# cxm12/TGSR

Measured on AMD Instinct MI355X. Metric: SR images/sec (32->256, batch 16 per GPU, one step in flight), higher is better.
Workload: dtype f32

## Files before the change

include/tgsr_hip.h:

```cpp
#ifndef TGSR_HIP_H
#define TGSR_HIP_H

#include <stdint.h>

#ifdef __cplusplus
extern "C" {
#endif

#define TGSR_OK 0
#define TGSR_EINVAL (-1)
#define TGSR_EUNSUPPORTED (-2)
#define TGSR_ELAUNCH (-3)

#define TGSR_EPI_AFFINE 0
#define TGSR_EPI_AFFINE_GLU 1

#define TGSR_ACT_NONE 0
#define TGSR_ACT_TANH_AXPY 1
#define TGSR_ACT_IDENT_AXPY 2

#define TGSR_ABI_VERSION 2
int tgsr_abi_version(void);
const char* tgsr_last_error(void);

int64_t tgsr_packed_weight_elems(int Cout, int Cin, int K);
int tgsr_pack_conv_weight(const float* w, float* wpack, int Cout, int Cin, int K, void* stream);
int tgsr_pack_conv_weight_dgrad(const float* w, float* wpack, int Cout, int Cin, int K, void* stream);

int tgsr_bn_fold(const float* weight, const float* bias, const float* running_mean, const float* running_var,
                 float eps, float* scale, float* shift, int C, void* stream);

int tgsr_conv3x3_fwd(const float* x, int64_t x_bstride, int B, int Cin, int H, int W, const float* wpack, int Cout,
                     const float* scale, const float* shift, const float* residual, int64_t res_bstride, float* out,
                     int64_t out_bstride, int epilogue, int upsample, void* stream);
int tgsr_conv3x3_fwd_plan(int B, int H, int W, int Cout, int epilogue, int upsample, int* nob, int* rows_per_wave, int* groups);

int64_t tgsr_packed_upconv_weight_elems(int Cout, int Cin);
int tgsr_pack_upconv_weight(const float* w, float* wpack, int Cout, int Cin, void* stream);
int tgsr_upconv3x3_glu_fwd(const float* x, int64_t x_bstride, int B, int Cin, int H, int W, const float* wpack, int Cout,
                           const float* scale, const float* shift, float* out, int64_t out_bstride, void* stream);

int64_t tgsr_packed_upwino_weight_elems(int Cout, int Cin);
int tgsr_pack_upwino_weight(const float* w, float* upack, int Cout, int Cin, int glu, void* stream);
int tgsr_upwino_glu_fwd(const float* x, int64_t x_bstride, int B, int Cin, int H, int W, const float* upack, int Cout,
                        const float* scale, const float* shift, float* out, int64_t out_bstride, void* stream);
int tgsr_upwino_fwd(const float* x, int64_t x_bstride, int B, int Cin, int H, int W, const float* upack, int Cout,
                    const float* scale, const float* shift, float* out, int64_t out_bstride, void* stream);

int64_t tgsr_packed_upwino4_weight_elems(int Cout, int Cin);
int tgsr_pack_upwino4_weight(const float* w, float* upack, int Cout, int Cin, int glu, void* stream);
int tgsr_upwino4_fwd(const float* x, int64_t x_bstride, int B, int Cin, int H, int W, const float* upack, int Cout,
                     const float* scale, const float* shift, float* out, int64_t out_bstride, int glu, void* stream);

int64_t tgsr_packed_wino_weight_elems(int Cout, int Cin);
int tgsr_pack_wino_weight(const float* w, float* upack, int Cout, int Cin, int glu, void* stream);
int tgsr_pack_wino_weight_dgrad(const float* w, float* upack, int Cout, int Cin, void* stream);
int tgsr_wino_conv3x3_fwd(const float* x, int64_t x_bstride, int B, int Cin, int H, int W, const float* upack, int Cout,
                          const float* scale, const float* shift, const float* residual, int64_t res_bstride,
                          float* out, int64_t out_bstride, int epilogue, void* stream);

int64_t tgsr_packed_wino4_weight_elems(int Cout, int Cin);
int tgsr_pack_wino4_weight(const float* w, float* upack, int Cout, int Cin, int glu, void* stream);
int tgsr_pack_wino4_weight_dgrad(const float* w, float* upack, int Cout, int Cin, void* stream);
int tgsr_wino4_conv3x3_fwd(const float* x, int64_t x_bstride, int B, int Cin, int H, int W, const float* upack, int Cout,
                           const float* scale, const float* shift, const float* residual, int64_t res_bstride,
                           float* out, int64_t out_bstride, int epilogue, void* stream);

int tgsr_pack_wino4_wide_weight(const float* w, float* upack, int Cout, int Cin, int glu, void* stream);
int tgsr_pack_wino4_wide_weight_dgrad(const float* w, float* upack, int Cout, int Cin, void* stream);
int tgsr_wino4_wide_stats_nslots(int B, int H, int W, int Cout);
int tgsr_wino4_wide_conv3x3_stats_fwd(const float* x, int64_t x_bstride, int B, int Cin, int H, int W, const float* upack,
                                      int Cout, float* out, int64_t out_bstride, float* stat_partial, void* stream);
int tgsr_wino4_wide_conv3x3_fwd(const float* x, int64_t x_bstride, int B, int Cin, int H, int W, const float* upack, int Cout,
                                const float* scale, const float* shift, const float* residual, int64_t res_bstride,
                                float* out, int64_t out_bstride, int epilogue, void* stream);

int tgsr_conv_to3_set_pipe(int on);

int tgsr_conv_to3_fwd(const float* x, int64_t x_bstride, int B, int Cin, int H, int W, const float* w, int K,
                      int act, const float* addend, float alpha, float* out, void* stream);
#define TGSR_TO3_FORM_MFMA 0
#define TGSR_TO3_FORM_PIPE 1
#define TGSR_TO3_FORM_VEC4 2
#define TGSR_TO3_FORM_SCALAR 3
int tgsr_conv_to3_plan(const float* x, int64_t x_bstride, int B, int Cin, int H, int W, int K, const float* addend,
                       const float* out, int* form, int* tile_rows);

int tgsr_conv_to3_finish_fwd(const float* x, int64_t x_bstride, int B, int Cin, int H, int W, const float* w, int K, float* out,
                             int n, float* const* fine, const float* const* t, const float* const* s, const int64_t* numel,
                             float alpha, void* stream);

int tgsr_word_attention_fwd(const float* h, int64_t h_bstride, const float* words, const float* w_ctx,
                            const uint8_t* mask, int mask_mode, int B, int idf, int cdf, int T, int Q, float* src_ws,
                            float* c_code, int64_t c_bstride, float* attn, void* stream);

int tgsr_word_project_fwd(const float* words, const float* const* w_ctx, int nsets, int B, int idf, int cdf, int T,
                          float* src_out, void* stream);

int tgsr_bilstm_fwd(const int64_t* captions, int width, const int32_t* cap_lens, int B, int Tmax, const float* emb,
                    int ntoken, int ninput, const float* w_ih, const float* w_hh, const float* b_ih,
                    const float* b_hh, int H, float* gates_ws, float* words_emb, float* sent_emb, void* stream);

int tgsr_lstm_gate_table(const float* emb, int ntoken, int ninput, const float* w_ih, const float* b_ih,
                         const float* b_hh, int H, float* table, void* stream);
int tgsr_bilstm_table_fwd(const int64_t* captions, int width, const int32_t* cap_lens, int B, int Tmax,
                          const float* table, int ntoken, const float* w_hh, int H, float* words_emb, float* sent_emb,
                          void* stream);

int tgsr_gru_gate_table(const float* emb, int ntoken, int ninput, const float* w_ih, const float* b_ih, const float* b_hh_rz,
                        int H, float* table, void* stream);
int tgsr_bigru_table_fwd(const int64_t* captions, int width, const int32_t* cap_lens, int B, int Tmax, const float* table,
                         int ntoken, const float* w_hh, const float* b_hn, int H, float* words_emb, float* sent_emb,
                         void* stream);

int tgsr_bigru_train_fwd(const float* x, const int32_t* cap_lens, int B, int Tmax, int ninput, const float* w_ih,
                         const float* w_hh, const float* b_ih, const float* b_hh_rz, const float* b_hn, int H, float* gates_ws,
                         float* acts, float* words_emb, float* sent_emb, void* stream);
int tgsr_bigru_bwd(const int32_t* cap_lens, int B, int Tmax, int H, const float* w_hh, const float* acts, const float* words_emb,
                   const float* d_words, const float* d_sent, float* dgx, float* dgh, float* hprev, float* dbias, void* stream);

int tgsr_bilstm_train_fwd(const float* x, const int32_t* cap_lens, int B, int Tmax, int ninput, const float* w_ih,
                          const float* w_hh, const float* b_ih, const float* b_hh, int H, float* gates_ws, float* acts,
                          float* words_emb, float* sent_emb, void* stream);
int tgsr_bilstm_bwd(const int32_t* cap_lens, int B, int Tmax, int H, const float* w_hh, const float* acts,
                    const float* words_emb, const float* d_words, const float* d_sent, float* dgates, float* hprev,
                    float* dbias, void* stream);

int tgsr_damsm_words_fwd(const float* words, const int32_t* cap_lens, const float* ctx, int B, int ndf, int Tw, int S,
                         float gamma1, float gamma2, float* sim, float* att_diag, void* stream);

int64_t tgsr_damsm_words_bwd_ws_elems(int B, int ndf, int S);
int tgsr_damsm_words_bwd(const float* words, const int32_t* cap_lens, const float* ctx, const float* grad_sim, int B,
                         int ndf, int Tw, int S, float gamma1, float gamma2, float* ws, float* grad_words32,
                         float* grad_ctx, void* stream);

int tgsr_func_attention_fwd(const float* query, const float* context, int B, int ndf, int L, int S, float gamma1,
                            float* weighted_context, float* attn, void* stream);

int tgsr_conv1x1_fwd(const float* x, int B, int Cin, int S, const float* w, const float* bias, int Cout, float* out,
                     void* stream);
int tgsr_linear_fwd(const float* x, int B, int K, const float* w, const float* bias, int Cout, float* out,
                    void* stream);
// ... 253 lines not shown
```

tgsr_amd/_lib.py:

```python
import ctypes
import os
import subprocess

_HERE = os.path.dirname(os.path.abspath(__file__))
LIB_PATH = os.environ.get("TGSR_LIB_PATH") or os.path.join(_HERE, "lib", "libtgsr_hip.so")
ABI_VERSION = 2

OK, EINVAL, EUNSUPPORTED, ELAUNCH = 0, -1, -2, -3
EPI_AFFINE, EPI_AFFINE_GLU = 0, 1
ACT_NONE, ACT_TANH_AXPY, ACT_IDENT_AXPY = 0, 1, 2
TO3_FORM_MFMA, TO3_FORM_PIPE, TO3_FORM_VEC4, TO3_FORM_SCALAR = 0, 1, 2, 3
DT_BF16, DT_F16 = 1, 2
WGRAD_DIRECT, WGRAD_WINO, WGRAD_UPWINO = 0, 1, 2
WGRAD_FAMILIES = ("conv3x3_wgrad_kernel<%d,%d,%s>", "wino_wgrad_kernel<%d,%d>", "wino_wgrad_dma_kernel<%d>", "upwino_wgrad_kernel<%d>")
WGRAD_PLAN_FIELDS, WGRAD_PLAN_WS = 10, 9
TO3_BWD_PLAN_FIELDS, TO3_BWD_PLAN_WS = 4, 3

_vp, _i, _i64, _f, _d = ctypes.c_void_p, ctypes.c_int, ctypes.c_int64, ctypes.c_float, ctypes.c_double

SIGNATURES = {
    "tgsr_abi_version": (_i, []),
    "tgsr_last_error": (ctypes.c_char_p, []),
    "tgsr_packed_weight_elems": (_i64, [_i, _i, _i]),
    "tgsr_pack_conv_weight": (_i, [_vp, _vp, _i, _i, _i, _vp]),
    "tgsr_pack_conv_weight_dgrad": (_i, [_vp, _vp, _i, _i, _i, _vp]),
    "tgsr_bn_fold": (_i, [_vp, _vp, _vp, _vp, _f, _vp, _vp, _i, _vp]),
    "tgsr_conv3x3_fwd": (_i, [_vp, _i64, _i, _i, _i, _i, _vp, _i, _vp, _vp, _vp, _i64, _vp, _i64, _i, _i, _vp]),
    "tgsr_conv3x3_fwd_plan": (_i, [_i, _i, _i, _i, _i, _i, _vp, _vp, _vp]),
    "tgsr_packed_upconv_weight_elems": (_i64, [_i, _i]),
    "tgsr_pack_upconv_weight": (_i, [_vp, _vp, _i, _i, _vp]),
    "tgsr_upconv3x3_glu_fwd": (_i, [_vp, _i64, _i, _i, _i, _i, _vp, _i, _vp, _vp, _vp, _i64, _vp]),
    "tgsr_packed_upwino_weight_elems": (_i64, [_i, _i]),
    "tgsr_pack_upwino_weight": (_i, [_vp, _vp, _i, _i, _i, _vp]),
    "tgsr_upwino_glu_fwd": (_i, [_vp, _i64, _i, _i, _i, _i, _vp, _i, _vp, _vp, _vp, _i64, _vp]),
    "tgsr_upwino_fwd": (_i, [_vp, _i64, _i, _i, _i, _i, _vp, _i, _vp, _vp, _vp, _i64, _vp]),
    "tgsr_packed_upwino4_weight_elems": (_i64, [_i, _i]),
    "tgsr_pack_upwino4_weight": (_i, [_vp, _vp, _i, _i, _i, _vp]),
    "tgsr_upwino4_fwd": (_i, [_vp, _i64, _i, _i, _i, _i, _vp, _i, _vp, _vp, _vp, _i64, _i, _vp]),
    "tgsr_packed_wino_weight_elems": (_i64, [_i, _i]),
    "tgsr_pack_wino_weight": (_i, [_vp, _vp, _i, _i, _i, _vp]),
    "tgsr_pack_wino_weight_dgrad": (_i, [_vp, _vp, _i, _i, _vp]),
    "tgsr_wino_conv3x3_fwd": (_i, [_vp, _i64, _i, _i, _i, _i, _vp, _i, _vp, _vp, _vp, _i64, _vp, _i64, _i, _vp]),
    "tgsr_packed_wino4_weight_elems": (_i64, [_i, _i]),
    "tgsr_pack_wino4_weight": (_i, [_vp, _vp, _i, _i, _i, _vp]),
    "tgsr_pack_wino4_weight_dgrad": (_i, [_vp, _vp, _i, _i, _vp]),
    "tgsr_pack_wino4_wide_weight": (_i, [_vp, _vp, _i, _i, _i, _vp]),
    "tgsr_pack_wino4_wide_weight_dgrad": (_i, [_vp, _vp, _i, _i, _vp]),
    "tgsr_wino4_wide_stats_nslots": (_i, [_i, _i, _i, _i]),
    "tgsr_wino4_wide_conv3x3_stats_fwd": (_i, [_vp, _i64, _i, _i, _i, _i, _vp, _i, _vp, _i64, _vp, _vp]),
    "tgsr_wino4_wide_conv3x3_fwd": (_i, [_vp, _i64, _i, _i, _i, _i, _vp, _i, _vp, _vp, _vp, _i64, _vp, _i64, _i, _vp]),
    "tgsr_wino4_conv3x3_fwd": (_i, [_vp, _i64, _i, _i, _i, _i, _vp, _i, _vp, _vp, _vp, _i64, _vp, _i64, _i, _vp]),
    "tgsr_conv_to3_fwd": (_i, [_vp, _i64, _i, _i, _i, _i, _vp, _i, _i, _vp, _f, _vp, _vp]),
    "tgsr_conv_to3_plan": (_i, [_vp, _i64, _i, _i, _i, _i, _i, _vp, _vp, _vp, _vp]),
    "tgsr_word_attention_fwd": (_i, [_vp, _i64, _vp, _vp, _vp, _i, _i, _i, _i, _i, _i, _vp, _vp, _i64, _vp, _vp]),
    "tgsr_word_project_fwd": (_i, [_vp, _vp, _i, _i, _i, _i, _i, _vp, _vp]),
    "tgsr_bilstm_fwd": (_i, [_vp, _i, _vp, _i, _i, _vp, _i, _i, _vp, _vp, _vp, _vp, _i, _vp, _vp, _vp, _vp]),
    "tgsr_lstm_gate_table": (_i, [_vp, _i, _i, _vp, _vp, _vp, _i, _vp, _vp]),
    "tgsr_bilstm_table_fwd": (_i, [_vp, _i, _vp, _i, _i, _vp, _i, _vp, _i, _vp, _vp, _vp]),
    "tgsr_bilstm_train_fwd": (_i, [_vp, _vp, _i, _i, _i, _vp, _vp, _vp, _vp, _i, _vp, _vp, _vp, _vp, _vp]),
    "tgsr_bilstm_bwd": (_i, [_vp, _i, _i, _i, _vp, _vp, _vp, _vp, _vp, _vp, _vp, _vp, _vp]),
    "tgsr_damsm_words_fwd": (_i, [_vp, _vp, _vp, _i, _i, _i, _i, _f, _f, _vp, _vp, _vp]),
    "tgsr_damsm_words_bwd_ws_elems": (_i64, [_i, _i, _i]),
    "tgsr_damsm_words_bwd": (_i, [_vp, _vp, _vp, _vp, _i, _i, _i, _i, _f, _f, _vp, _vp, _vp, _vp]),
    "tgsr_func_attention_fwd": (_i, [_vp, _vp, _i, _i, _i, _i, _f, _vp, _vp, _vp]),
    "tgsr_conv1x1_fwd": (_i, [_vp, _i, _i, _i, _vp, _vp, _i, _vp, _vp]),
    "tgsr_linear_fwd": (_i, [_vp, _i, _i, _vp, _vp, _i, _vp, _vp]),
    "tgsr_rowdot_fwd": (_i, [_vp, _vp, _vp, _vp, _i, _i, _vp]),
    "tgsr_ca_net_fwd": (_i, [_vp, _vp, _vp, _vp, _i, _i, _i, _vp, _vp, _vp, _vp]),
    "tgsr_rowdot_bwd": (_i, [_vp, _vp, _vp, _vp, _vp, _i, _i, _vp]),
    "tgsr_bn_train_nsplit": (_i, [_i, _i, _i]),
    "tgsr_bn_train_fwd": (_i, [_vp, _i, _i, _i, _vp, _vp, _f, _f, _vp, _vp, _i, _vp, _i64, _vp, _vp, _vp, _vp, _vp, _vp,
                               _i64, _vp, _vp]),
    "tgsr_bn_train_bwd": (_i, [_vp, _vp, _i, _i, _i, _vp, _vp, _vp, _vp, _i, _vp, _vp, _vp, _vp, _vp, _vp]),
    "tgsr_dconv_set_split": (_i, [_i]),
    "tgsr_bn_set_fuse_small": (_i, [_i]),
    "tgsr_conv_to3_set_pipe": (_i, [_i]),
    "tgsr_conv_to3_finish_fwd": (_i, [_vp, _i64, _i, _i, _i, _i, _vp, _i, _vp, _i, _vp, _vp, _vp, _vp, _f, _vp]),
    "tgsr_conv4x4s2_split_form": (_i, [_i, _i, _i, _i, _i, _i]),
    "tgsr_conv3x3_gemm_split_form": (_i, [_i, _i, _i, _i, _i, _i]),
    "tgsr_conv4x4s2_ws_elems": (_i64, [_i, _i, _i, _i, _i, _i]),
    "tgsr_conv4x4s2_fwd": (_i, [_vp, _i, _i, _i, _i, _vp, _i, _i, _vp, _vp, _vp]),
    "tgsr_conv4x4s2_dgrad": (_i, [_vp, _i, _i, _i, _i, _vp, _i, _vp, _vp, _vp]),
    "tgsr_conv4x4s2_wgrad": (_i, [_vp, _vp, _i, _i, _i, _i, _i, _vp, _vp, _vp]),
    "tgsr_conv3x3_gemm_ws_elems": (_i64, [_i, _i, _i, _i, _i, _i]),
    "tgsr_conv3x3_gemm_fwd": (_i, [_vp, _i, _i, _i, _i, _vp, _i, _vp, _vp, _vp]),
    "tgsr_conv3x3_gemm_dgrad": (_i, [_vp, _i, _i, _i, _i, _vp, _i, _vp, _vp, _vp]),
    "tgsr_conv3x3_gemm_wgrad": (_i, [_vp, _vp, _i, _i, _i, _i, _i, _vp, _vp, _vp]),
    "tgsr_leaky_relu": (_i, [_vp, _vp, _vp, _i64, _vp]),
    "tgsr_glu": (_i, [_vp, _vp, _vp, _i64, _i64, _vp]),
    "tgsr_wino_stats_nslots": (_i, [_i, _i, _i, _i]),
    "tgsr_wino_conv3x3_stats_fwd": (_i, [_vp, _i64, _i, _i, _i, _i, _vp, _i, _vp, _i64, _vp, _vp]),
    "tgsr_wino4_stats_nslots": (_i, [_i, _i, _i, _i]),
    "tgsr_wino4_conv3x3_stats_fwd": (_i, [_vp, _i64, _i, _i, _i, _i, _vp, _i, _vp, _i64, _vp, _vp]),
    "tgsr_bn_train_fwd_from_stats": (_i, [_vp, _i, _i, _i, _vp, _vp, _f, _f, _vp, _vp, _i, _vp, _i64, _vp, _i, _vp, _vp, _vp, _vp,
                                          _vp, _i64, _vp, _vp]),
    "tgsr_text_tail_fwd": (_i, [_vp, _vp, _i, _i, _i, _i, _i, _vp, _vp, _vp, _vp, _i, _i, _vp, _vp, _vp, _i, _vp, _vp]),
    "tgsr_gru_gate_table": (_i, [_vp, _i, _i, _vp, _vp, _vp, _i, _vp, _vp]),
    "tgsr_bigru_table_fwd": (_i, [_vp, _i, _vp, _i, _i, _vp, _i, _vp, _vp, _i, _vp, _vp, _vp]),
    "tgsr_bigru_train_fwd": (_i, [_vp, _vp, _i, _i, _i, _vp, _vp, _vp, _vp, _vp, _i, _vp, _vp, _vp, _vp, _vp]),
    "tgsr_bigru_bwd": (_i, [_vp, _i, _i, _i, _vp, _vp, _vp, _vp, _vp, _vp, _vp, _vp, _vp, _vp]),
    "tgsr_lp_att_pack_bytes": (_i64, [_i, _i]),
    "tgsr_text_tail_lp_fwd": (_i, [_vp, _vp, _i, _i, _i, _i, _i, _vp, _vp, _vp, _vp, _i, _i, _vp, _vp, _vp, _i, _vp, _i, _vp, _vp]),
    "tgsr_lp_stem_att_fwd": (_i, [_i, _vp, _i, _i, _i, _vp, _i, _vp, _vp, _vp, _i, _i, _vp, _i, _i, _i, _i, _i, _i, _vp, _vp]),
    "tgsr_lp_upconv_glu_att_fwd": (_i, [_i, _vp, _i, _i, _i, _i, _i, _vp, _i, _vp, _vp, _vp, _i, _i, _vp, _i, _vp, _vp, _i, _i,
                                        _i, _i, _i, _i, _vp, _vp]),
    "tgsr_multi_copy": (_i, [_i, _vp, _vp, _vp, _vp]),
    "tgsr_axpy_images": (_i, [_i, _vp, _vp, _vp, _vp, _f, _vp]),
    "tgsr_gconv_set_form": (_i, [_i]),
    "tgsr_gconv_nsplit": (_i, [_i, _i, _i]),
    "tgsr_gconv_ws_elems": (_i64, [_i, _i, _i, _i, _i]),
    "tgsr_gconv": (_i, [_i, _vp, _vp, _i64, _i, _i, _i, _i, _i, _i, _i, _i, _i, _i, _i, _i, _vp, _i, _i, _vp, _vp, _i64, _vp, _vp]),
    "tgsr_gconv_pack": (_i, [_vp, _vp, _vp, _i, _i, _i, _i, _vp]),
    "tgsr_gconv_stats_nslots": (_i, [_i, _i, _i, _i, _i]),
    "tgsr_gconv_stats_slot_pixels": (_i, [_i, _i, _i, _i, _i]),
    "tgsr_gconv_stats": (_i, [_vp, _vp, _i64, _i, _i, _i, _i, _i, _i, _i, _i, _i, _i, _i, _i, _vp, _i64, _vp, _vp, _vp]),
    "tgsr_bn_train_relu_slice_from_stats": (_i, [_vp, _i64, _i, _i, _i, _vp, _vp, _f, _f, _vp, _vp, _vp, _i, _i, _vp, _vp, _vp]),
    "tgsr_maxpool3s2_fwd": (_i, [_vp, _i64, _i, _i, _i, _i, _vp, _i64, _vp]),
    "tgsr_maxpool3s2_bwd": (_i, [_vp, _i64, _vp, _i64, _i, _i, _i, _i, _vp, _i64, _i, _vp, _vp]),
    "tgsr_avgpool3": (_i, [_vp, _i64, _i, _i, _i, _i, _vp, _i64, _i, _vp, _vp]),
    "tgsr_sum_stack": (_i, [_vp, _i, _i64, _vp, _vp]),
    "tgsr_interleave2x2": (_i, [_vp, _vp, _vp, _vp, _vp, _i64, _i, _i, _i, _vp, _vp]),
    "tgsr_plane_mean": (_i, [_vp, _vp, _i64, _i, _vp]),
    "tgsr_plane_mean_bwd": (_i, [_vp, _vp, _i64, _i, _vp]),
    "tgsr_relu_mask": (_i, [_vp, _i64, _vp, _i64, _vp, _i64, _i, _i64, _vp]),
    "tgsr_bilinear_fwd": (_i, [_vp, _i64, _i, _i, _i, _i, _vp, _vp]),
# ... 106 lines not shown
```

tgsr_amd/csrc/tgsr_winograd.hip:

```cpp
#include "tgsr_common.h"

#include <cstdlib>
#include <type_traits>

namespace tgsr {

typedef __attribute__((address_space(3))) void* lds_ptrw_t;
typedef const __attribute__((address_space(1))) void* glb_ptrw_t;
__device__ __attribute__((aligned(16))) float g_wino_zero[4] = {0.f, 0.f, 0.f, 0.f};

#ifdef TGSR_WINO_STAMPS
__device__ unsigned long long g_wstamps[8 * 8192];
#define TGSR_WSTAMP(k)                                                                                  \
  do {                                                                                                  \
    const int bid_ = blockIdx.x;                                                                        \
    if (threadIdx.x == 0 && bid_ < 8192) {                                                              \
      g_wstamps[bid_ * 8 + (k)] = __builtin_amdgcn_s_memtime();                                         \
      if ((k) == 0) g_wstamps[bid_ * 8 + 6] = __builtin_amdgcn_s_memrealtime();                         \
      if ((k) == 3) g_wstamps[bid_ * 8 + 7] = __builtin_amdgcn_s_memrealtime();                         \
    }                                                                                                   \
  } while (0)
#else
#define TGSR_WSTAMP(k)
#endif
// ... 263 lines not shown
  if (NH == 2 && h) run(std::integral_constant<int, 1>{});
  else run(std::integral_constant<int, 0>{});
  TGSR_WSTAMP(2);

  auto ytile = [&](int cb, int i, float (&y)[2][2]) {
    float rr[4][2];
#pragma unroll
    for (int r = 0; r < 4; ++r) {
      const float m0 = M[r * 4 + 0][cb][i], m1 = M[r * 4 + 1][cb][i], m2 = M[r * 4 + 2][cb][i], m3 = M[r * 4 + 3][cb][i];
      rr[r][0] = m0 + m1 + m2;
      rr[r][1] = m1 - m2 - m3;
    }
#pragma unroll
    for (int dx = 0; dx < 2; ++dx) {
      y[0][dx] = rr[0][dx] + rr[1][dx] + rr[2][dx];
      y[1][dx] = rr[1][dx] - rr[2][dx] - rr[3][dx];
    }
  };
  float ssum[2][4] = {{0.f, 0.f, 0.f, 0.f}, {0.f, 0.f, 0.f, 0.f}}, ssq[2][4] = {{0.f, 0.f, 0.f, 0.f}, {0.f, 0.f, 0.f, 0.f}};
  if (ox < a.W) {
    if (GLU) {
#pragma unroll
      for (int i = 0; i < 4; ++i) {
        const int lc = h * 32 + 4 * lg + i;
        float yv[2][2], yg[2][2];
        ytile(0, i, yv);
        ytile(1, i, yg);
        const float sv = aff_s[lc], tv = aff_s[64 + lc], sg = aff_s[lc + 16], tg = aff_s[64 + lc + 16];
        const int c = grp * (16 * NH) + h * 16 + 4 * lg + i;
#pragma unroll
        for (int dy = 0; dy < 2; ++dy) {
          if (oy + dy >= a.H) continue;
          const float o0 = (yv[dy][0] * sv + tv) * __builtin_amdgcn_rcpf(1.f + __expf(-(yg[dy][0] * sg + tg)));
          const float o1 = (yv[dy][1] * sv + tv) * __builtin_amdgcn_rcpf(1.f + __expf(-(yg[dy][1] * sg + tg)));
          *reinterpret_cast<float2*>(ob + (int64_t)c * HWo + (int64_t)(oy + dy) * a.W + ox) = make_float2(o0, o1);
        }
      }
    } else {
#pragma unroll
      for (int cb = 0; cb < 2; ++cb) {
#pragma unroll
        for (int i = 0; i < 4; ++i) {
          const int lc = h * 32 + cb * 16 + 4 * lg + i;
          float yv[2][2];
          ytile(cb, i, yv);
          const float sv = aff_s[lc], tv = aff_s[64 + lc];
#pragma unroll
          for (int dy = 0; dy < 2; ++dy) {
            if (oy + dy >= a.H) continue;
            const float o0 = yv[dy][0] * sv + tv + rres[cb][i][dy].x, o1 = yv[dy][1] * sv + tv + rres[cb][i][dy].y;
            *reinterpret_cast<float2*>(ob + (int64_t)(grp * (32 * NH) + lc) * HWo + (int64_t)(oy + dy) * a.W + ox) =
                make_float2(o0, o1);
            if (STATS) {
              ssum[cb][i] += o0 + o1;
              ssq[cb][i] += o0 * o0 + o1 * o1;
            }
          }
        }
      }
    }
  }
  if (STATS) {
    const int slot = ((b * a.tiles_y + ty) * a.tiles_x + tx) * Geo::ROWS + w;
#pragma unroll
    for (int cb = 0; cb < 2; ++cb) {
#pragma unroll
      for (int i = 0; i < 4; ++i) {
        float s = ssum[cb][i], q = ssq[cb][i];
#pragma unroll
        for (int o = 8; o >= 1; o >>= 1) {
          s += __shfl_xor(s, o);
          q += __shfl_xor(q, o);
        }
        if (l15 == 0) {
          const int c = grp * (32 * NH) + h * 32 + cb * 16 + 4 * lg + i;
          *reinterpret_cast<float2*>(a.stat + ((int64_t)c * a.nslots + slot) * 2) = make_float2(s, q);
        }
      }
    }
  }
  TGSR_WSTAMP(3);
}

__global__ void pack_wino_weight_kernel(const float* __restrict__ w, float* __restrict__ up, int Cout, int Cin, int glu,
                                        int nh, int tr, int64_t total) {
  const int ngrp = Cout / (32 * nh);
  for (int64_t idx = (int64_t)blockIdx.x * blockDim.x + threadIdx.x; idx < total; idx += (int64_t)gridDim.x * blockDim.x) {
    const int q = (int)(idx & 3), l = (int)((idx >> 2) & 15), hh = nh == 2 ? (int)((idx >> 6) & 1) : 0;
    int64_t t = idx >> (nh == 2 ? 7 : 6);
    const int ci = (int)(t % kWCK);
    t /= kWCK;
    const int pp = (int)(t % 8);
    t /= 8;
    const int grp = (int)(t % ngrp);
    const int st = (int)(t / ngrp);
    const int pos = 2 * pp + (q >> 1), cb = q & 1;
    const int co = glu ? (cb ? (Cout >> 1) : 0) + grp * (16 * nh) + hh * 16 + l
                       : grp * (32 * nh) + hh * 32 + cb * 16 + l;
    const int c = st * kWCK + ci;
    float u = 0.f;
    if (c < Cin) {
      const int i = pos >> 2, j = pos & 3;
      const float* g = tr ? w + ((int64_t)c * Cout + co) * 9 : w + ((int64_t)co * Cin + c) * 9;
      float gi[3];
      for (int k = 0; k < 3; ++k) {
        const float g0 = tr ? g[8 - k] : g[0 * 3 + k], g1 = tr ? g[5 - k] : g[1 * 3 + k], g2 = tr ? g[2 - k] : g[2 * 3 + k];
        gi[k] = i == 0 ? g0 : (i == 1 ? 0.5f * (g0 + g1 + g2) : (i == 2 ? 0.5f * (g0 - g1 + g2) : g2));
      }
      u = j == 0 ? gi[0] : (j == 1 ? 0.5f * (gi[0] + gi[1] + gi[2]) : (j == 2 ? 0.5f * (gi[0] - gi[1] + gi[2]) : gi[2]));
    }
    up[idx] = u;
  }
}

}

using namespace tgsr;

#ifdef TGSR_WINO_STAMPS
extern "C" int tgsr_debug_read_wstamps(unsigned long long* host, int n) {
  return hipMemcpyFromSymbol(host, HIP_SYMBOL(tgsr::g_wstamps), sizeof(unsigned long long) * n) == hipSuccess ? 0 : -3;
}
#endif

extern "C" int64_t tgsr_packed_wino_weight_elems(int Cout, int Cin) {
  return (int64_t)((Cin + kWCK - 1) / kWCK) * 16 * kWCK * Cout;
}

static int pack_wino_weight(const float* w, float* upack, int Cout, int Cin, int glu, int tr, void* stream) {
  if (!w || !upack || Cout < 1 || Cin < 1) return TGSR_EINVAL;
  if (Cout % 32 != 0) return TGSR_EUNSUPPORTED;
  const int64_t total = tgsr_packed_wino_weight_elems(Cout, Cin);
  const int blocks = (int)((total + 255) / 256 < 2048 ? (total + 255) / 256 : 2048);
  hipLaunchKernelGGL(pack_wino_weight_kernel, dim3(blocks), dim3(256), 0, as_stream(stream), w, upack, Cout, Cin,
                     glu ? 1 : 0, Cout % 64 == 0 ? 2 : 1, tr, total);
  return note_launch(hipGetLastError(), "pack_wino_weight_kernel");
}

extern "C" int tgsr_pack_wino_weight(const float* w, float* upack, int Cout, int Cin, int glu, void* stream) {
  return pack_wino_weight(w, upack, Cout, Cin, glu, 0, stream);
}

extern "C" int tgsr_pack_wino_weight_dgrad(const float* w, float* upack, int Cout, int Cin, void* stream) {
  return pack_wino_weight(w, upack, Cout, Cin, 0, 1, stream);
}

static void wino_geometry(int B, int Cin, int H, int W, int Cout, WinoArgs& a) {
  const int nh = Cout % 64 == 0 ? 2 : 1;
  a.tiles_x = (W + 31) / 32; a.tiles_y = nh == 2 ? (H + 3) / 4 : (H + 7) / 8; a.nstages = (Cin + kWCK - 1) / kWCK;
  a.ngroups = Cout / (32 * nh);
  a.nslots = B * a.tiles_y * a.tiles_x * (nh == 2 ? 2 : 4);
}

extern "C" int tgsr_wino_stats_nslots(int B, int H, int W, int Cout) {
  if (B < 1 || H < 1 || W < 1 || Cout < 1 || Cout % 32 != 0) return 0;
  WinoArgs a;
  wino_geometry(B, 4, H, W, Cout, a);
  return a.nslots;
}

static int wino_conv3x3(const float* x, int64_t x_bstride, int B, int Cin, int H, int W, const float* upack, int Cout,
                        const float* scale, const float* shift, const float* residual, int64_t res_bstride, float* out,
                        int64_t out_bstride, int epilogue, float* stat, void* stream) {
  if (!x || !upack || !out || B < 1 || Cin < 1 || H < 1 || W < 1 || Cout < 1) return TGSR_EINVAL;
  if ((scale == nullptr) != (shift == nullptr)) return TGSR_EINVAL;
  const bool glu = epilogue == TGSR_EPI_AFFINE_GLU;
  if (!glu && epilogue != TGSR_EPI_AFFINE) return TGSR_EINVAL;
  if (glu && residual) return TGSR_EINVAL;
  if (Cout % 32 != 0 || Cin % kWCK != 0) return TGSR_EUNSUPPORTED;
  if ((int64_t)H * W >= (1 << 28) || (int64_t)Cin * H * W >= (1ll << 32)) return TGSR_EUNSUPPORTED;
  if ((W & 3) || (x_bstride & 3) || (reinterpret_cast<uintptr_t>(x) & 15) || (reinterpret_cast<uintptr_t>(out) & 7) || (out_bstride & 1) ||
      (residual && ((reinterpret_cast<uintptr_t>(residual) & 7) || (res_bstride & 1))))
    return TGSR_EUNSUPPORTED;
  WinoArgs a;
  a.x = x; a.xbs = x_bstride; a.B = B; a.Cin = Cin; a.H = H; a.W = W; a.upack = upack; a.Cout = Cout;
  a.scale = scale; a.shift = shift; a.res = residual; a.rbs = res_bstride; a.out = out; a.obs = out_bstride;
  const int nh = Cout % 64 == 0 ? 2 : 1;
  wino_geometry(B, Cin, H, W, Cout, a);
  a.stat = stat;
  if (stat && (glu || residual || scale)) return TGSR_EINVAL;
  dim3 grid((unsigned)(B * a.tiles_x * a.tiles_y * a.ngroups));
  size_t dyn = 0;
#ifdef TGSR_WINO_STAMPS
  if (const char* e = getenv("TGSR_WINO_DYN")) dyn = (size_t)atoi(e);
#endif
  if (nh == 2) {
    if (glu) hipLaunchKernelGGL((wino_conv3x3_kernel<true, 2>), grid, dim3(256), dyn, as_stream(stream), a);
    else if (stat) hipLaunchKernelGGL((wino_conv3x3_kernel<false, 2, true>), grid, dim3(256), dyn, as_stream(stream), a);
    else hipLaunchKernelGGL((wino_conv3x3_kernel<false, 2>), grid, dim3(256), dyn, as_stream(stream), a);
  } else {
    if (glu) hipLaunchKernelGGL((wino_conv3x3_kernel<true, 1>), grid, dim3(256), dyn, as_stream(stream), a);
    else if (stat) hipLaunchKernelGGL((wino_conv3x3_kernel<false, 1, true>), grid, dim3(256), dyn, as_stream(stream), a);
    else hipLaunchKernelGGL((wino_conv3x3_kernel<false, 1>), grid, dim3(256), dyn, as_stream(stream), a);
  }
  return note_launch(hipGetLastError(), "wino_conv3x3_kernel");
}

extern "C" int tgsr_wino_conv3x3_fwd(const float* x, int64_t x_bstride, int B, int Cin, int H, int W,
                                     const float* upack, int Cout, const float* scale, const float* shift,
                                     const float* residual, int64_t res_bstride, float* out, int64_t out_bstride,
                                     int epilogue, void* stream) {
  return wino_conv3x3(x, x_bstride, B, Cin, H, W, upack, Cout, scale, shift, residual, res_bstride, out, out_bstride,
                      epilogue, nullptr, stream);
}

extern "C" int tgsr_wino_conv3x3_stats_fwd(const float* x, int64_t x_bstride, int B, int Cin, int H, int W,
                                           const float* upack, int Cout, float* out, int64_t out_bstride,
                                           float* stat_partial, void* stream) {
  if (!stat_partial) return TGSR_EINVAL;
  return wino_conv3x3(x, x_bstride, B, Cin, H, W, upack, Cout, nullptr, nullptr, nullptr, 0, out, out_bstride,
                      TGSR_EPI_AFFINE, stat_partial, stream);
}
```

tgsr_amd/ops.py:

```python
import collections
import ctypes
import functools
import os
from typing import Optional, Tuple

import torch

from . import _lib
from ._lib import TgsrError, check

BN_EPS = 1e-5

profile = None


def _ev():
    e = torch.cuda.Event(enable_timing=True)
    e.record()
    return e


_raw_stream = getattr(torch._C, "_cuda_getCurrentRawStream", None)


# ... 725 lines not shown

def func_attention(query: torch.Tensor, context: torch.Tensor, gamma1: float):
    _need_hip(query, context)
    B, ndf, L = query.shape
    ih, iw = context.shape[2], context.shape[3]
    q = _f32(query, "query").contiguous()
    c = _f32(context, "context").contiguous()
    wc = torch.empty(B, ndf, L, dtype=torch.float32, device=q.device)
    attn = torch.empty(B, L, ih, iw, dtype=torch.float32, device=q.device)
    rc = _lib.lib().tgsr_func_attention_fwd(_p(q), _p(c), B, ndf, L, ih * iw, float(gamma1), _p(wc), _p(attn),
                                            _stream())
    check(rc, "tgsr_func_attention_fwd")
    return wc, attn


CONV1X1_GCONV = os.environ.get("TGSR_CONV1X1_GCONV", "1") != "0"


def conv1x1(x: torch.Tensor, w: torch.Tensor, bias: Optional[torch.Tensor] = None) -> torch.Tensor:
    _need_hip(x, w, bias)
    x = _f32(x, "x").contiguous()
    B, Cin, H, W = x.shape
    w2 = _f32(w.detach(), "w").reshape(w.shape[0], -1).contiguous()
    if w2.shape[1] != Cin:
        raise TgsrError("conv1x1: weight %s vs input channels %d" % (tuple(w.shape), Cin))
    out = torch.empty(B, w2.shape[0], H, W, dtype=torch.float32, device=x.device)
    if bias is None and Cin % 16 == 0 and B * H * W >= 1024 and CONV1X1_GCONV:
        need = gconv_ws_elems(B, w2.shape[0], H, W, Cin)
        ws = torch.empty(need, dtype=torch.float32, device=x.device) if need else None
        gconv(False, w2, x, 0, Cin, out, 0, 1, 1, 1, 0, 0, None, False, False, ws, None)
        return out
    b = None if bias is None else _f32(bias.detach(), "bias").contiguous()
    check(_lib.lib().tgsr_conv1x1_fwd(_p(x), B, Cin, H * W, _p(w2), _p(b), w2.shape[0], _p(out), _stream()),
          "tgsr_conv1x1_fwd")
    return out


def conv1x1_wgrad(dy: torch.Tensor, x: torch.Tensor) -> Optional[torch.Tensor]:
    _need_hip(dy, x)
    B, Cout, H, W = dy.shape
    Cin, K = x.shape[1], B * H * W
    if not CONV1X1_GCONV or K % 16 != 0 or K < 1024 or Cin < 64 or tuple(x.shape) != (B, Cin, H, W):
        return None
    a = _f32(dy, "dy").permute(1, 0, 2, 3).reshape(Cout, K).contiguous()
    xt = _f32(x, "x").permute(0, 2, 3, 1).reshape(1, K, Cin, 1).contiguous()
    out = torch.empty(1, Cout, Cin, 1, dtype=torch.float32, device=dy.device)
    need = gconv_ws_elems(1, Cout, Cin, 1, K)
    ws = torch.empty(need, dtype=torch.float32, device=dy.device) if need else None
    gconv(False, a, xt, 0, K, out, 0, 1, 1, 1, 0, 0, None, False, False, ws, None)
    return out.reshape(Cout, Cin)


def linear(x: torch.Tensor, w: torch.Tensor, bias: Optional[torch.Tensor] = None) -> torch.Tensor:
    _need_hip(x, w, bias)
    x = _f32(x, "x").contiguous()
    w2 = _f32(w.detach(), "w").contiguous()
    B, K = x.shape
    if w2.shape[1] != K:
        raise TgsrError("linear: weight %s vs input %s" % (tuple(w.shape), tuple(x.shape)))
    b = None if bias is None else _f32(bias.detach(), "bias").contiguous()
    if CONV1X1_GCONV and K % 16 == 0 and K >= 256:
        xt = x.t().contiguous().view(1, K, B, 1)
        img = torch.empty(1, w2.shape[0], B, 1, dtype=torch.float32, device=x.device)
        need = gconv_ws_elems(1, w2.shape[0], B, 1, K)
        ws = torch.empty(need, dtype=torch.float32, device=x.device) if need else None
        gconv(False, w2, xt, 0, K, img, 0, 1, 1, 1, 0, 0, b, False, False, ws, None)
        return img.view(w2.shape[0], B).t().contiguous()
    out = torch.empty(B, w2.shape[0], dtype=torch.float32, device=x.device)
    check(_lib.lib().tgsr_linear_fwd(_p(x), B, K, _p(w2), _p(b), w2.shape[0], _p(out), _stream()), "tgsr_linear_fwd")
    return out


def conv_to3_set_pipe(on: bool) -> bool:
    return bool(_lib.lib().tgsr_conv_to3_set_pipe(1 if on else 0))


def conv_to3_pipe() -> bool:
    L = _lib.lib()
    was = L.tgsr_conv_to3_set_pipe(1)
    L.tgsr_conv_to3_set_pipe(was)
    return bool(was)


def bn_set_fuse_small(on: bool) -> bool:
    return bool(_lib.lib().tgsr_bn_set_fuse_small(1 if on else 0))


def bn_train_fwd(raw: torch.Tensor, gamma: torch.Tensor, beta: torch.Tensor, eps: float, momentum: float,
                 running_mean: Optional[torch.Tensor], running_var: Optional[torch.Tensor], act: int = 0,
                 residual: Optional[torch.Tensor] = None, nbt: Optional[torch.Tensor] = None,
                 out: Optional[torch.Tensor] = None, stats: Optional[torch.Tensor] = None,
                 stat_partial: Optional[torch.Tensor] = None):
    _need_hip(raw, gamma, beta, running_mean, running_var, residual, nbt, out, stats, stat_partial)
    L = _lib.lib()
    B, C, Ho, Wo = raw.shape
    HW, dev = Ho * Wo, raw.device
    raw = _f32(raw, "raw")
    if not raw.is_contiguous():
        raise TgsrError("bn_train_fwd: raw must be contiguous")
    co = C // 2 if act == 1 else C
    if out is None:
        out = torch.empty(B, co, Ho, Wo, dtype=torch.float32, device=dev)
    if stats is None:
        stats = torch.empty(4, C, dtype=torch.float32, device=dev)
    res = None if residual is None else residual.contiguous()
    if stat_partial is not None:
        if (stat_partial.dim() != 3 or stat_partial.shape[0] != C or stat_partial.shape[2] != 2 or
                stat_partial.dtype != torch.float32 or not stat_partial.is_contiguous()):
            raise TgsrError("bn_train_fwd: stat_partial %s for %d channels" % (tuple(stat_partial.shape), C))
        s0, s1, s2, s3 = _rows4(stats)
        rc = L.tgsr_bn_train_fwd_from_stats(_p(raw), B, C, HW, _p(gamma), _p(beta), float(eps),
                                            float(momentum), _p(running_mean), _p(running_var), int(act), _p(res),
                                            0 if res is None else co * HW, _p(stat_partial), stat_partial.shape[1],
                                            s0, s1, s2, s3, _p(out), co * HW, _p(nbt), _stream())
        check(rc, "tgsr_bn_train_fwd_from_stats")
        return out, stats
    ws = torch.empty(C * L.tgsr_bn_train_nsplit(B, C, HW) * 4, dtype=torch.float32, device=dev)
    s0, s1, s2, s3 = _rows4(stats)
    rc = L.tgsr_bn_train_fwd(_p(raw), B, C, HW, _p(gamma), _p(beta), float(eps), float(momentum),
                             _p(running_mean), _p(running_var), int(act), _p(res), 0 if res is None else co * HW, _p(ws),
                             s0, s1, s2, s3, _p(out), co * HW, _p(nbt), _stream())
    check(rc, "tgsr_bn_train_fwd")
    return out, stats


def bn_train_bwd(dout: torch.Tensor, raw: torch.Tensor, stats: torch.Tensor, act: int, dgamma: Optional[torch.Tensor] = None,
                 dbeta: Optional[torch.Tensor] = None, draw: Optional[torch.Tensor] = None):
    _need_hip(dout, raw, stats, dgamma, dbeta, draw)
    L = _lib.lib()
    B, C, Ho, Wo = raw.shape
    HW, dev = Ho * Wo, raw.device
    dout = _f32(dout, "dout").contiguous()
    co = C // 2 if act == 1 else C
    if draw is None:
        draw = torch.empty_like(raw)
    if dgamma is None:
        dgamma = torch.empty(C, dtype=torch.float32, device=dev)
    if dbeta is None:
        dbeta = torch.empty(C, dtype=torch.float32, device=dev)
    ws = torch.empty(co * L.tgsr_bn_train_nsplit(B, co, HW) * 4, dtype=torch.float32, device=dev)
    s0, s1, s2, s3 = _rows4(stats)
    rc = L.tgsr_bn_train_bwd(_p(dout), _p(raw), B, C, HW, s2, s3, s0, s1, int(act),
                             _p(ws), _p(ws), _p(draw), _p(dgamma), _p(dbeta), _stream())
    check(rc, "tgsr_bn_train_bwd")
    return draw, dgamma, dbeta


def sumpool2x2(x: torch.Tensor) -> torch.Tensor:
    _need_hip(x)
    x = _f32(x, "x").contiguous()
    B, C, H2, W2 = x.shape
    out = torch.empty(B, C, H2 // 2, W2 // 2, dtype=torch.float32, device=x.device)
    check(_lib.lib().tgsr_sumpool2x2(_p(x), B * C, H2 // 2, W2 // 2, _p(out), _stream()), "tgsr_sumpool2x2")
    return out


def conv3x3_wgrad_kind(Cin: int, Cout: int, upsample: bool, winograd: bool = True) -> str:
    if winograd and Cin % 32 == 0:
        if upsample:
            return "upwino" if Cout % 64 == 0 else "direct"
        if Cout % 32 == 0:
            return "wino"
    return "direct"


_WGRAD = {"direct": ("tgsr_conv3x3_wgrad", "conv3x3_wgrad_kernel"), "wino": ("tgsr_wino_wgrad", "wino_wgrad_kernel"),
# ... 896 lines not shown
```

Measured before the change: 12570.

## Add 512-thread split Winograd conv kernel for under-filled grids

Adds a Winograd 3x3 forward kernel variant that uses 512 threads per block, splitting the accumulation work across twice as many waves (qh halves) and exchanging partial results through LDS in the epilogue. It is selected automatically when the tile-group grid is smaller than two rounds of CUs, targeting the low-occupancy small-image layers of this workload. Adds a runtime mode switch and an env override. Costs extra LDS exchange and barriers, and the kernel has higher register and LDS pressure per block.

```diff
diff --git a/include/tgsr_hip.h b/include/tgsr_hip.h
--- a/include/tgsr_hip.h
+++ b/include/tgsr_hip.h
@@ -58,6 +58,8 @@
 int tgsr_wino_conv3x3_fwd(const float* x, int64_t x_bstride, int B, int Cin, int H, int W, const float* upack, int Cout,
                           const float* scale, const float* shift, const float* residual, int64_t res_bstride,
                           float* out, int64_t out_bstride, int epilogue, void* stream);
+int tgsr_wino_split_wanted(int B, int Cin, int H, int W, int Cout, int stats, int cus);
+int tgsr_wino_set_split(int mode);
 
 int64_t tgsr_packed_wino4_weight_elems(int Cout, int Cin);
 int tgsr_pack_wino4_weight(const float* w, float* upack, int Cout, int Cin, int glu, void* stream);
diff --git a/tgsr_amd/_lib.py b/tgsr_amd/_lib.py
--- a/tgsr_amd/_lib.py
+++ b/tgsr_amd/_lib.py
@@ -41,6 +41,8 @@
     "tgsr_pack_wino_weight": (_i, [_vp, _vp, _i, _i, _i, _vp]),
     "tgsr_pack_wino_weight_dgrad": (_i, [_vp, _vp, _i, _i, _vp]),
     "tgsr_wino_conv3x3_fwd": (_i, [_vp, _i64, _i, _i, _i, _i, _vp, _i, _vp, _vp, _vp, _i64, _vp, _i64, _i, _vp]),
+    "tgsr_wino_split_wanted": (_i, [_i, _i, _i, _i, _i, _i, _i]),
+    "tgsr_wino_set_split": (_i, [_i]),
     "tgsr_packed_wino4_weight_elems": (_i64, [_i, _i]),
     "tgsr_pack_wino4_weight": (_i, [_vp, _vp, _i, _i, _i, _vp]),
     "tgsr_pack_wino4_weight_dgrad": (_i, [_vp, _vp, _i, _i, _vp]),
diff --git a/tgsr_amd/csrc/tgsr_winograd.hip b/tgsr_amd/csrc/tgsr_winograd.hip
--- a/tgsr_amd/csrc/tgsr_winograd.hip
+++ b/tgsr_amd/csrc/tgsr_winograd.hip
@@ -369,6 +369,283 @@
   TGSR_WSTAMP(3);
 }
 
+template <bool GLU>
+__global__ __launch_bounds__(512, 2) void wino_conv3x3_split_kernel(WinoArgs a) {
+  using Geo = WinoGeo<2>;
+  constexpr int kWPLANE = Geo::PLANE, kWU = Geo::U, kWRawN = Geo::RAWN, kWRaw = Geo::RAW;
+  constexpr int kWUK = kWU / 512 / 4;
+  static_assert(Geo::RP == 4 && kWUK == 2, "waves 0..3 copy the raw tile, every wave two pieces of U");
+  static_assert(8 * 1024 <= 3 * kWU, "the epilogue's exchange (8 waves x 64 lanes x 16 floats) fits the U region");
+  __shared__ __attribute__((aligned(16))) float smem[Geo::SMEM];
+  const int tid = threadIdx.x, lane = tid & 63, l15 = lane & 15, lg = lane >> 4;
+  const int wave = __builtin_amdgcn_readfirstlane(tid >> 6);
+  const int qh = wave >> 2, w = (wave >> 1) & 1, h = wave & 1;
+  int t = xcd_remap(blockIdx.x, gridDim.x);
+  const int grp = t % a.ngroups;
+  t /= a.ngroups;
+  const int tx = t % a.tiles_x;
+  t /= a.tiles_x;
+  const int ty = t % a.tiles_y;
+  const int b = t / a.tiles_y;
+  const int y0 = ty * (2 * Geo::ROWS), x0 = tx * 32;
+  const float* xb = a.x + (int64_t)b * a.xbs;
+  const uint32_t HW = (uint32_t)a.H * (uint32_t)a.W;
+  float* us = smem;
+  float* raws = smem + 3 * kWU;
+  float* vs = smem + 3 * kWU + 3 * kWRaw + w * 2 * kWV;
+  float* aff_s = smem + 3 * kWU + 3 * kWRaw + Geo::ROWS * 2 * kWV;
+  TGSR_WSTAMP(0);
+
+  const float* rptr;
+  int rstep;
+  {
+    const int e = ((wave & 3) * 64 + lane) * 4;
+    const int c = e / kWPLANE;
+    const int rem = e - c * kWPLANE;
+    const int r = rem / kWTC, j = rem - r * kWTC;
+    const int gy = y0 - 1 + r, gx = x0 - 4 + j;
+    const bool ok = e < kWRawN && (unsigned)gy < (unsigned)a.H && (unsigned)gx < (unsigned)a.W;
+    rptr = ok ? xb + (uint64_t)(uint32_t)c * HW + (uint32_t)(gy * a.W + gx) : g_wino_zero;
+    rstep = ok ? (int)(kWCK * HW) : 0;
+  }
+  auto issue_raw = [&](int buf) {
+    if (!qh) {
+      const unsigned l = __builtin_amdgcn_readfirstlane((unsigned)(size_t)(lds_ptrw_t)(raws + buf * kWRaw + wave * 256));
+      asm volatile("s_mov_b32 m0, %1\n\ts_nop 0\n\tglobal_load_lds_dwordx4 %0, off" ::"v"(rptr), "s"(l) : "memory");
+      rptr += rstep;
+    }
+  };
+  const float* ubase = a.upack + (int64_t)grp * kWU;
+  const int64_t ustride = (int64_t)a.ngroups * kWU;
+  unsigned uoff[kWUK];
+#pragma unroll
+  for (int k = 0; k < kWUK; ++k) uoff[k] = (unsigned)(((wave + 8 * k) * 64 + lane) * 16);
+  auto issue_u = [&](int buf) {
+#pragma unroll
+    for (int k = 0; k < kWUK; ++k) {
+      const unsigned l = __builtin_amdgcn_readfirstlane((unsigned)(size_t)(lds_ptrw_t)(us + buf * kWU + (wave + 8 * k) * 256));
+      asm volatile("s_mov_b32 m0, %2\n\ts_nop 0\n\tglobal_load_lds_dwordx4 %0, %1" ::"v"(uoff[k]), "s"(ubase), "s"(l)
+                   : "memory");
+    }
+    ubase += ustride;
+  };
+
+  const int rlane = lg * kWPLANE + (2 * w) * kWTC + 2 * l15 + 3;
+  const int vwl0 = lg * 32 + l15 * 2;
+  auto t_read = [&](auto ic, const float* rawb, float (&d)[2][4]) {
+    constexpr int I = decltype(ic)::value;
+    constexpr int rowA = I == 0 ? 0 : (I == 2 ? 2 : 1), rowB = I == 3 ? 3 : (I == 2 ? 1 : 2);
+    const float* rp = rawb + rlane;
+#pragma unroll
+    for (int c = 0; c < 4; ++c) {
+      d[0][c] = rp[rowA * kWTC + c];
+      d[1][c] = rp[rowB * kWTC + c];
+    }
+  };
+  auto t_write = [&](auto ic, const float (&d)[2][4], float* vdst) {
+    constexpr int I = decltype(ic)::value;
+    float tr[4];
+#pragma unroll
+    for (int c = 0; c < 4; ++c) tr[c] = I == 1 ? d[0][c] + d[1][c] : d[0][c] - d[1][c];
+    float* vp = vdst + vwl0 + (2 * I) * (kWCK * 32);
+    *reinterpret_cast<float2*>(vp) = make_float2(tr[0] - tr[2], tr[1] + tr[2]);
+    *reinterpret_cast<float2*>(vp + kWCK * 32) = make_float2(tr[2] - tr[1], tr[1] - tr[3]);
+  };
+  auto with_row = [&](auto f) {
+    if (h) {
+      if (qh) f(std::integral_constant<int, 3>{});
+      else f(std::integral_constant<int, 2>{});
+    } else {
+      if (qh) f(std::integral_constant<int, 1>{});
+      else f(std::integral_constant<int, 0>{});
+    }
+  };
+
+  if (tid < 128) {
+    const int lc = tid & 63, hh = lc >> 5, cb = (lc >> 4) & 1, l = lc & 15;
+    int col = GLU ? (cb ? (a.Cout >> 1) : 0) + grp * 32 + hh * 16 + l : grp * 64 + lc;
+    if (col >= a.Cout) col = 0;
+    aff_s[tid] = a.scale ? (tid < 64 ? a.scale[col] : a.shift[col]) : (tid < 64 ? 1.f : 0.f);
+  }
+
+  f32x4v M[8][2];
+#pragma unroll
+  for (int p = 0; p < 8; ++p)
+#pragma unroll
+    for (int cb = 0; cb < 2; ++cb)
+#pragma unroll
+      for (int i = 0; i < 4; ++i) M[p][cb][i] = 0.f;
+
+  issue_raw(0);
+  issue_u(0);
+  if (a.nstages > 1) { issue_raw(1); issue_u(1); }
+  if (a.nstages > 2) issue_raw(2);
+  asm volatile("s_waitcnt vmcnt(0) lgkmcnt(0)\n\ts_barrier" ::: "memory");
+  with_row([&](auto ic) {
+    float d[2][4];
+    t_read(ic, raws, d);
+    t_write(ic, d, vs);
+  });
+  __syncthreads();
+  TGSR_WSTAMP(1);
+
+  const int ulane = qh * 4 * (kWCK * 2 * 64) + (lg * 2 + h) * 64 + l15 * 4;
+  const int vlane = qh * 4 * (kWCK * 32) + lg * 32 + l15 * 2;
+  const int oy = y0 + 2 * w, ox = x0 + 2 * l15;
+  const int64_t HWo = (int64_t)a.H * a.W;
+  float* __restrict__ ob = a.out + (int64_t)b * a.obs;
+  const float* __restrict__ rb = a.res ? a.res + (int64_t)b * a.rbs : nullptr;
+  float2 rres[4][2];
+  auto load_res = [&]() {
+    if (!GLU) {
+#pragma unroll
+      for (int i = 0; i < 4; ++i)
+#pragma unroll
+        for (int dy = 0; dy < 2; ++dy) {
+          rres[i][dy] = make_float2(0.f, 0.f);
+          if (rb && ox < a.W && oy + dy < a.H)
+            rres[i][dy] = *reinterpret_cast<const float2*>(
+                rb + (int64_t)(grp * 64 + h * 32 + qh * 16 + 4 * lg + i) * HWo + (int64_t)(oy + dy) * a.W + ox);
+        }
+    }
+  };
+
+  int b3 = 0;
+  auto stage = [&](auto ic, auto more_c, auto more2_c, auto more3_c, int st) {
+    constexpr bool MORE = decltype(more_c)::value, MORE2 = decltype(more2_c)::value, MORE3 = decltype(more3_c)::value;
+    const int par = st & 1;
+    const int b3n = b3 == 2 ? 0 : b3 + 1, b3p = b3 == 0 ? 2 : b3 - 1;
+    const float* ub = us + b3 * kWU + ulane;
+    const float* vb = vs + par * kWV + vlane;
+    f32x4v af[4];
+    float2 bf[4];
+    float d[2][4];
+#pragma unroll
+    for (int j = 0; j < 4; ++j) {
+      af[j] = *reinterpret_cast<const f32x4v*>(ub + j * kWCK * 2 * 64);
+      bf[j] = *reinterpret_cast<const float2*>(vb + j * kWCK * 32);
+      __builtin_amdgcn_sched_barrier(0);
+    }
+    if (MORE) t_read(ic, raws + b3n * kWRaw, d);
+    __builtin_amdgcn_sched_barrier(0);
+#pragma unroll
+    for (int j = 0; j < 4; ++j) {
+      M[2 * j][0] = __builtin_amdgcn_mfma_f32_16x16x4f32(af[j][0], bf[j].x, M[2 * j][0], 0, 0, 0);
+      M[2 * j][1] = __builtin_amdgcn_mfma_f32_16x16x4f32(af[j][1], bf[j].x, M[2 * j][1], 0, 0, 0);
+      M[2 * j + 1][0] = __builtin_amdgcn_mfma_f32_16x16x4f32(af[j][2], bf[j].y, M[2 * j + 1][0], 0, 0, 0);
+      M[2 * j + 1][1] = __builtin_amdgcn_mfma_f32_16x16x4f32(af[j][3], bf[j].y, M[2 * j + 1][1], 0, 0, 0);
+      if (j < 3) {
+        __builtin_amdgcn_sched_barrier(0);
+        if (j == 0 && MORE2) issue_u(b3p);
+        if (j == 1 && MORE) {
+          asm volatile("" : "+v"(d[0][0]), "+v"(d[0][1]), "+v"(d[0][2]), "+v"(d[0][3]), "+v"(d[1][0]), "+v"(d[1][1]), "+v"(d[1][2]),
+                            "+v"(d[1][3]));
+          t_write(ic, d, vs + (par ^ 1) * kWV);
+        }
+        if (j == 2 && MORE3) issue_raw(b3);
+        __builtin_amdgcn_sched_barrier(0);
+      }
+    }
+    if (MORE) {
+      constexpr int kU = MORE2 ? kWUK : 0;
+      if (MORE3 && !qh) asm volatile("s_waitcnt vmcnt(%0) lgkmcnt(0)\n\ts_barrier" ::"n"(kU + 1) : "memory");
+      else asm volatile("s_waitcnt vmcnt(%0) lgkmcnt(0)\n\ts_barrier" ::"n"(kU) : "memory");
+    }
+    b3 = b3n;
+  };
+
+  auto finish = [&](auto qc) {
+    constexpr int Q = decltype(qc)::value;
+    float rr[2][2][4][2];
+#pragma unroll
+    for (int rl = 0; rl < 2; ++rl)
+#pragma unroll
+      for (int cb = 0; cb < 2; ++cb)
+#pragma unroll
+        for (int i = 0; i < 4; ++i) {
+          const float m0 = M[rl * 4 + 0][cb][i], m1 = M[rl * 4 + 1][cb][i], m2 = M[rl * 4 + 2][cb][i], m3 = M[rl * 4 + 3][cb][i];
+          rr[rl][cb][i][0] = m0 + m1 + m2;
+          rr[rl][cb][i][1] = m1 - m2 - m3;
+        }
+    asm volatile("s_waitcnt lgkmcnt(0)\n\ts_barrier" ::: "memory");
+    float* xw = us + (((w * 2 + h) * 2 + Q) * 4) * 256 + lane * 4;
+    const float* xr = us + (((w * 2 + h) * 2 + (Q ^ 1)) * 4) * 256 + lane * 4;
+#pragma unroll
+    for (int s = 0; s < 4; ++s) {
+      constexpr int F = Q ^ 1;
+      const int cb = GLU ? s >> 1 : F, i = GLU ? 2 * F + (s & 1) : s;
+      f32x4v v;
+      v[0] = rr[0][cb][i][0]; v[1] = rr[0][cb][i][1]; v[2] = rr[1][cb][i][0]; v[3] = rr[1][cb][i][1];
+      *reinterpret_cast<f32x4v*>(xw + s * 256) = v;
+    }
+    asm volatile("s_waitcnt lgkmcnt(0)\n\ts_barrier" ::: "memory");
+    float yy[4][2][2];
+#pragma unroll
+    for (int s = 0; s < 4; ++s) {
+      const int cb = GLU ? s >> 1 : Q, i = GLU ? 2 * Q + (s & 1) : s;
+      const f32x4v o = *reinterpret_cast<const f32x4v*>(xr + s * 256);
+      float r4[4][2];
+#pragma unroll
+      for (int dx = 0; dx < 2; ++dx) {
+        r4[2 * Q][dx] = rr[0][cb][i][dx];
+        r4[2 * Q + 1][dx] = rr[1][cb][i][dx];
+        r4[2 * (Q ^ 1)][dx] = o[dx];
+        r4[2 * (Q ^ 1) + 1][dx] = o[2 + dx];
+      }
+#pragma unroll
+      for (int dx = 0; dx < 2; ++dx) {
+        yy[s][0][dx] = r4[0][dx] + r4[1][dx] + r4[2][dx];
+        yy[s][1][dx] = r4[1][dx] - r4[2][dx] - r4[3][dx];
+      }
+    }
+    if (ox >= a.W) return;
+    if (GLU) {
+#pragma unroll
+      for (int ii = 0; ii < 2; ++ii) {
+        const int i = 2 * Q + ii;
+        const int lc = h * 32 + 4 * lg + i;
+        const float (&yv)[2][2] = yy[ii];
+        const float (&yg)[2][2] = yy[2 + ii];
+        const float sv = aff_s[lc], tv = aff_s[64 + lc], sg = aff_s[lc + 16], tg = aff_s[64 + lc + 16];
+        const int c = grp * 32 + h * 16 + 4 * lg + i;
+#pragma unroll
+        for (int dy = 0; dy < 2; ++dy) {
+          if (oy + dy >= a.H) continue;
+          const float o0 = (yv[dy][0] * sv + tv) * __builtin_amdgcn_rcpf(1.f + __expf(-(yg[dy][0] * sg + tg)));
+          const float o1 = (yv[dy][1] * sv + tv) * __builtin_amdgcn_rcpf(1.f + __expf(-(yg[dy][1] * sg + tg)));
+          *reinterpret_cast<float2*>(ob + (int64_t)c * HWo + (int64_t)(oy + dy) * a.W + ox) = make_float2(o0, o1);
+        }
+      }
+    } else {
+#pragma unroll
+      for (int i = 0; i < 4; ++i) {
+        const int lc = h * 32 + Q * 16 + 4 * lg + i;
+        const float (&yv)[2][2] = yy[i];
+        const float sv = aff_s[lc], tv = aff_s[64 + lc];
+#pragma unroll
+        for (int dy = 0; dy < 2; ++dy) {
+          if (oy + dy >= a.H) continue;
+          const float o0 = yv[dy][0] * sv + tv + rres[i][dy].x, o1 = yv[dy][1] * sv + tv + rres[i][dy].y;
+          *reinterpret_cast<float2*>(ob + (int64_t)(grp * 64 + lc) * HWo + (int64_t)(oy + dy) * a.W + ox) = make_float2(o0, o1);
+        }
+      }
+    }
+  };
+  with_row([&](auto ic) {
+    using T = std::true_type;
+    using F = std::false_type;
+    int st = 0;
+    for (; st + 3 < a.nstages; ++st) stage(ic, T{}, T{}, T{}, st);
+    if (st + 2 < a.nstages) stage(ic, T{}, T{}, F{}, st++);
+    if (st + 1 < a.nstages) stage(ic, T{}, F{}, F{}, st++);
+    load_res();
+    stage(ic, F{}, F{}, F{}, st);
+    TGSR_WSTAMP(2);
+    finish(std::integral_constant<int, decltype(ic)::value & 1>{});
+  });
+  TGSR_WSTAMP(3);
+}
+
 __global__ void pack_wino_weight_kernel(const float* __restrict__ w, float* __restrict__ up, int Cout, int Cin, int glu,
                                         int nh, int tr, int64_t total) {
   const int ngrp = Cout / (32 * nh);
@@ -444,6 +721,44 @@
   WinoArgs a;
   wino_geometry(B, 4, H, W, Cout, a);
   return a.nslots;
+}
+
+static int g_wino_split = [] {
+  const char* e = getenv("TGSR_WINO_SPLIT");
+  const int v = e ? atoi(e) : 2;
+  return v < 0 || v > 2 ? 2 : v;
+}();
+
+constexpr int kWinoSplitRounds = 2;
+
+extern "C" int tgsr_wino_set_split(int mode) {
+  if (mode < 0 || mode > 2) return TGSR_EINVAL;
+  const int was = g_wino_split;
+  g_wino_split = mode;
+  return was;
+}
+
+extern "C" int tgsr_wino_split_wanted(int B, int Cin, int H, int W, int Cout, int stats, int cus) {
+  if (B < 1 || Cin < 1 || H < 1 || W < 1 || Cout < 1 || cus < 1) return 0;
+  if (Cout % 64 != 0 || stats) return 0;
+  WinoArgs a;
+  wino_geometry(B, Cin, H, W, Cout, a);
+  return (int64_t)B * a.tiles_x * a.tiles_y * a.ngroups < (int64_t)kWinoSplitRounds * cus ? 1 : 0;
+}
+
+static int wino_device_cus() {
+  static int cus[64] = {0};
+  int dev = 0;
+  if (hipGetDevice(&dev) != hipSuccess || dev < 0 || dev >= 64) dev = 0;
+  if (cus[dev] < 1) {
+    int n = 0;
+    if (hipDeviceGetAttribute(&n, hipDeviceAttributeMultiprocessorCount, dev) != hipSuccess || n < 1) {
+      (void)hipGetLastError();
+      return 0;
+    }
+    cus[dev] = n;
+  }
+  return cus[dev];
 }
 
 static int wino_conv3x3(const float* x, int64_t x_bstride, int B, int Cin, int H, int W, const float* upack, int Cout,
@@ -471,7 +786,12 @@
 #ifdef TGSR_WINO_STAMPS
   if (const char* e = getenv("TGSR_WINO_DYN")) dyn = (size_t)atoi(e);
 #endif
-  if (nh == 2) {
+  const bool split = nh == 2 && !stat && g_wino_split != 0 &&
+                     (g_wino_split == 1 || tgsr_wino_split_wanted(B, Cin, H, W, Cout, 0, wino_device_cus()));
+  if (split) {
+    if (glu) hipLaunchKernelGGL((wino_conv3x3_split_kernel<true>), grid, dim3(512), dyn, as_stream(stream), a);
+    else hipLaunchKernelGGL((wino_conv3x3_split_kernel<false>), grid, dim3(512), dyn, as_stream(stream), a);
+  } else if (nh == 2) {
     if (glu) hipLaunchKernelGGL((wino_conv3x3_kernel<true, 2>), grid, dim3(256), dyn, as_stream(stream), a);
     else if (stat) hipLaunchKernelGGL((wino_conv3x3_kernel<false, 2, true>), grid, dim3(256), dyn, as_stream(stream), a);
     else hipLaunchKernelGGL((wino_conv3x3_kernel<false, 2>), grid, dim3(256), dyn, as_stream(stream), a);
diff --git a/tgsr_amd/ops.py b/tgsr_amd/ops.py
--- a/tgsr_amd/ops.py
+++ b/tgsr_amd/ops.py
@@ -831,6 +831,12 @@
     return bool(was)
 
 
+def wino_set_split(mode: int) -> int:
+    was = _lib.lib().tgsr_wino_set_split(int(mode))
+    check(min(was, 0), "tgsr_wino_set_split(%r)" % (mode,))
+    return was
+
+
 def bn_set_fuse_small(on: bool) -> bool:
     return bool(_lib.lib().tgsr_bn_set_fuse_small(1 if on else 0))
 
```

New measurement: 12510. Within noise of the previous version (-0.5%).
